# bcgsc/NanoSim

Measured on AMD Instinct MI355X. Metric: simulated reads/sec (genome mode, mean 8 kb), higher is better.
Workload: dtype u8

## Files before the change

### nanosim_amd/csrc/nanosim_amd.hip

```cpp
#include <hip/hip_runtime.h>
#include <hipcub/hipcub.hpp>
#include <stdio.h>
#include <stdlib.h>
#include <string.h>
#include <algorithm>
#include <chrono>
#include <atomic>
#include <condition_variable>
#include <functional>
#include <mutex>
#include <thread>
#include <string>
#include <vector>

#include "ns_device.h"
#include "ns_materialise.h"
#include "ns_chain.h"
#include "ns_hp.h"
#include "ns_ir.h"
#include "ns_io.h"
#include "ns_pack.h"
#include "ns_cs_hist.h"

#ifndef NS_WPB
// ... 1065 lines not shown
        const ns_piece p = A.pieces[gp];
        const uint32_t kind = uni(p.kind);
        const uint32_t out_len = (HPF && !kind) ? uni(A.hp_len[gp]) : uni(p.out_len);
        qualities_piece(A.m, Q, ro, key, a, kind ? NS_GAP_SEG + (pi >> 1) : (pi >> 1), kind, out_len, q, cls + (q >> 4) + 2u * pi, lane);
        q += out_len;
    }
    if (A.polya) {
        const uint32_t pl = uni(A.polya[r]);
        if (pl) emit_polya_quals(A.m, ro, key, a, q, pl, rd.head, rd.tail, lane);
    }
}

#define NS_DENSE_SEG 4096u
__global__ void __launch_bounds__(256) k_dense_plan(GenArgs A, uint32_t *cnt) {
    const uint64_t r = (uint64_t)blockIdx.x * blockDim.x + threadIdx.x;
    if (r > A.prm.n_reads) return;
    uint32_t c = 0;
    if (r < A.prm.n_reads) { const ns_read rd = A.reads[r]; c = rd.flags ? 0u : max(1u, (rd.seq_len + NS_DENSE_SEG - 1u) / NS_DENSE_SEG); }
    cnt[r] = c;
}
template <bool FASTQ>
__global__ void __launch_bounds__(64) k_materialise_dense(GenArgs A, const uint32_t *__restrict__ seg_off) {
    __shared__ DenseLds S;
    const uint32_t lane = threadIdx.x;
    const uint32_t w = blockIdx.x, n = (uint32_t)A.prm.n_reads;
    if (w >= seg_off[n]) return;
    uint32_t lo = 0, hi = n;
    while (hi - lo > 1) { const uint32_t mid = (lo + hi) >> 1; if (seg_off[mid] <= w) lo = mid; else hi = mid; }
    const uint64_t r = uni(lo);
    const uint32_t seg = uni(w - seg_off[lo]);
    ns_read rd; ns_key key; ReadOut ro;
    if (!load_read_uniform(A, r, FASTQ, rd, key, ro)) return;
    const uint32_t a = rd.attempts;
    if (seg == 0) emit_head_tail(A.m, ro, key, a, rd.head, rd.tail, lane);
    uint32_t q = rd.head;
    for (uint32_t pi = 0; pi < rd.n_pieces; ++pi) {
        const PieceCtx pc = load_piece_uniform(A.events, A.ref, A.pieces[rd.piece_off + pi], pi);
        const uint64_t s_lo = (uint64_t)seg * NS_DENSE_SEG, s_hi = s_lo + NS_DENSE_SEG, p_lo = q - rd.head, p_hi = p_lo + pc.out_len;
        if (p_hi > s_lo && p_lo < s_hi) {
            const uint32_t m_lo = (uint32_t)(max(s_lo, p_lo) - p_lo), m_hi = (uint32_t)(min(s_hi, p_hi) - p_lo);
            if (A.dbg & 16384u) slow_piece_range(A.m, A.ref, ro, key, a, pc, q, m_lo, m_hi, lane);
            else dense_piece<FASTQ>(A.m, A.ref, S, ro, key, a, pc, q, m_lo, m_hi, lane);
        }
        q += pc.out_len;
    }
}

template <bool FASTQ, bool SCRATCH>
__global__ void __launch_bounds__(64) k_materialise_slow(GenArgs A, SlowQueue sq) {
    const uint32_t lane = threadIdx.x;
    const uint32_t n = min(*sq.count, sq.cap);
    for (uint32_t i = blockIdx.x; i < n; i += gridDim.x) {
        const SlowTile t = sq.items[i];
        ns_read rd; ns_key key; ReadOut ro;
        if (!load_read_uniform(A, t.read, FASTQ && !SCRATCH, rd, key, ro)) continue;
        uint32_t q = SCRATCH ? 0u : rd.head;
        if constexpr (SCRATCH) { ro.seq = A.scr + A.scr_off[t.read]; ro.qual = nullptr; ro.reversed = false; ro.uracil = false; }
        for (uint32_t pi = 0; pi < t.piece; ++pi) q += A.pieces[rd.piece_off + pi].out_len;
        const PieceCtx pc = load_piece_uniform(A.events, A.ref, A.pieces[rd.piece_off + t.piece], t.piece);
        slow_piece_range<FASTQ && SCRATCH>(A.m, A.ref, ro, key, rd.attempts, pc, q, t.m0, t.m1, lane);
    }
}

template <bool FASTQ>
__global__ void __launch_bounds__(64) k_materialise_slow_hpf(GenArgs A, SlowQueue sq) {
    const uint32_t lane = threadIdx.x;
// ... 407 lines not shown
}

__global__ void __launch_bounds__(64 * NS_WPB) k_errlen(GenArgs A) {
    const uint32_t lane = threadIdx.x & 63;
    const uint64_t r = (uint64_t)blockIdx.x * (blockDim.x >> 6) + (threadIdx.x >> 6);
    if (r >= A.prm.n_reads) return;
    const ns_read rd = A.reads[r];
    unsigned long long sum = 0;
    if (!rd.flags) {
        const uint32_t nl = A.name_len[r];
        for (uint32_t pi = 0; pi < rd.n_pieces; ++pi) {
            const ns_piece p = A.pieces[rd.piece_off + pi];
            if (p.kind) continue;
            const ns_event *ev = A.events + p.ev_off;
            for (uint32_t j = lane; j < p.n_ev; j += 64) {
                const ns_event e = ev[j];
                sum += nl + dec_digits(e.pos) + dec_digits(ns_ev_len(e.info)) + 2u * ns_ev_len(e.info) + 9u;
            }
        }
    }
    sum = wave_sum(sum);
    if (lane == 0) A.err_len[r] = sum;
}

#define NS_ERR_BUF_SMALL 5120u
#define NS_ERR_BUF_LARGE 8192u
#define NS_ERR_PAD 16u
#define NS_ERR_NAME 256u
#define NS_ERR_NAME_ROW (NS_ERR_NAME + 8u)
template <uint32_t BUF>
__global__ void __launch_bounds__(64) k_errlog(GenArgs A) {
    __shared__ __align__(16) uint8_t buf_lds[NS_ERR_PAD + BUF + 16];
    __shared__ __align__(16) uint8_t name_lds[4][NS_ERR_NAME_ROW];
    const uint32_t lane = threadIdx.x & 63;
    const uint64_t r = blockIdx.x;
    if (r >= A.prm.n_reads) return;
    const ns_read rd = A.reads[r];
    if (rd.flags) return;
    const ns_key key = read_key(A, r);
    const uint32_t a = rd.attempts;
    const uint32_t nl = A.name_len[r];
    const uint8_t *name = A.records + rd.rec_off + 1;
    const bool name_in_lds = nl <= NS_ERR_NAME;
    if (name_in_lds) {
        for (uint32_t j = lane; 4u * j < nl + 4u; j += 64) {
            uint32_t v0 = 0;
            for (uint32_t b = 0; b < 4; ++b) if (4u * j + b < nl) v0 |= (uint32_t)name[4u * j + b] << (8 * b);
            const uint32_t vp = j ? (uint32_t)name[4u * j - 1] | (uint32_t)name[4u * j - 2] << 8 | (uint32_t)name[4u * j - 3] << 16 : 0u;
            *reinterpret_cast<uint32_t *>(&name_lds[0][4u * j]) = v0;
            *reinterpret_cast<uint32_t *>(&name_lds[1][4u * j]) = v0 << 8 | (vp & 0xffu);
            *reinterpret_cast<uint32_t *>(&name_lds[2][4u * j]) = v0 << 16 | (vp & 0xffu) << 8 | ((vp >> 8) & 0xffu);
            *reinterpret_cast<uint32_t *>(&name_lds[3][4u * j]) = v0 << 24 | (vp & 0xffu) << 16 | ((vp >> 8) & 0xffu) << 8 | (vp >> 16);
        }
        wave_sync();
    }
    uint64_t base = A.err_off[r];
    for (uint32_t pi = 0; pi < rd.n_pieces; pi += 2) {
        const ns_piece p = A.pieces[rd.piece_off + pi];
        PieceCtx pc = load_piece(A.events, A.ref, p, pi);
        ns_event e_nx; e_nx.pos = 0; e_nx.info = 0;
        if (lane < p.n_ev) e_nx = pc.ev[p.n_ev - 1 - lane];
        for (uint32_t j0 = 0; j0 < p.n_ev; j0 += 64) {
            const uint32_t k = j0 + lane;
            const bool active = k < p.n_ev;
            const ns_event e = e_nx;
            const uint32_t len = ns_ev_len(e.info), ty = ns_ev_type(e.info);
            const uint32_t tail = dec_digits(e.pos) + dec_digits(len) + 2u * len + 9u;
            const uint32_t row = active ? nl + tail : 0;
            const uint32_t incl = wave_incl_scan(row);
            const uint32_t total = (uint32_t)__builtin_amdgcn_readlane((int)incl, 63);
            const bool staged = name_in_lds && total <= BUF;
            auto fields = [&](auto w) __attribute__((always_inline)) {
                if (A.dbg & (1u << 17)) return;
                *w++ = '\t'; w = put_dec_p(w, e.pos); *w++ = '\t';
                const char *tn = ty == NS_MIS ? "mis" : ty == NS_INS ? "ins" : "del";
                *w++ = (uint8_t)tn[0]; *w++ = (uint8_t)tn[1]; *w++ = (uint8_t)tn[2];
                *w++ = '\t'; w = put_dec_p(w, len); *w++ = '\t';
                auto w2 = w + len + 1;
                if (A.dbg & (1u << 18)) return;
                const bool need_ref = ty != NS_INS;
                const bool inside = pc.pos + e.pos + 16ull <= pc.chrom_len;
                uint32_t r16[4] = {0x2d2d2d2du, 0x2d2d2d2du, 0x2d2d2d2du, 0x2d2d2d2du}, n16[4] = {0x2d2d2d2du, 0x2d2d2d2du, 0x2d2d2d2du, 0x2d2d2d2du};
                if (need_ref && inside) __builtin_memcpy(r16, A.ref.bases + pc.chrom_base + pc.pos + e.pos, 16);
                bool fast = len <= 16u && (!need_ref || inside);
                if (fast && need_ref) {
                    const uint32_t nb = 8u * (len & 3u), full = len >> 2;
                    uint32_t amb = 0;
#pragma unroll
                    for (uint32_t g = 0; g < 4; ++g) amb |= r16[g] & (g < full ? 0x80808080u : g == full ? (0x80808080u & ((1u << nb) - 1u)) : 0u);
                    fast = amb == 0;
                }
                if (ty != NS_DEL) {
                    const uint32_t word = payload_word(key, pc.sid, a, p.n_ev - 1 - k, 0);
                    uint32_t f3 = word;
#pragma unroll
                    for (uint32_t g = 0; g < 4; ++g) {
                        if (ty == NS_INS) {
                            const uint32_t x8 = (word >> (8u * g)) & 0xffu, t8 = (x8 | x8 << 12) & 0x000f000fu;
                            n16[g] = __builtin_amdgcn_perm(0u, 0x47435441u, (t8 | t8 << 6) & 0x03030303u);
                        } else {
                            const uint32_t d0 = next_digit3(f3), d1 = next_digit3(f3), d2 = next_digit3(f3), d3 = next_digit3(f3);
                            const uint32_t d4 = d0 | d1 << 8 | d2 << 16 | d3 << 24;
                            const uint32_t vv = (r16[g] >> 1) & 0x03030303u;
                            const uint32_t rank4 = (vv & 0x01010101u) << 1 | ((vv >> 1) & 0x01010101u);
                            const uint32_t ge = ((d4 | 0x80808080u) - rank4) & 0x80808080u;
                            n16[g] = __builtin_amdgcn_perm(0u, 0x47435441u, d4 + (ge >> 7));
                        }
                    }
                }
#pragma unroll
                for (uint32_t i = 0; i < 16; ++i) {
                    const bool on = fast && i < len;
                    if (!__ballot(on)) break;
                    if (on) { w[i] = (uint8_t)(r16[i >> 2] >> (8u * (i & 3u))); w2[i] = (uint8_t)(n16[i >> 2] >> (8u * (i & 3u))); }
                }
                if (!fast) {
                    uint32_t frac = 0;
                    for (uint32_t i = 0; i < len; ++i) {
                        if (ty != NS_DEL && !(i & 15u)) frac = payload_word(key, pc.sid, a, p.n_ev - 1 - k, i >> 4);
                        if (ty == NS_INS) { w[i] = '-'; w2[i] = bases_atcg((frac >> (2u * (i & 15u))) & 3u); }
                        else {
                            uint32_t x = e.pos + i;
                            uint8_t cur = resolve_base((uint32_t)ref_base_at(A.ref, pc, x), key, pc.sid, a, x);
                            w[i] = cur;
                            w2[i] = (ty == NS_MIS) ? mis_from_digit(cur, next_digit3(frac)) : (uint8_t)'-';
                        }
                    }
                }
                w[len] = '\t';
                w2[len] = '\n';
            };
            if (staged) {
                uint8_t *const dst0 = A.errlog + base;
                const uint32_t mis = (uint32_t)(uintptr_t)dst0 & 15u;
                if (active) {
// ... 344 lines not shown
    }
    uint32_t *hist = (uint32_t *)ctx->ord_bins.p, *cursor = hist + NS_ORD_BINS;
    const unsigned tiles = (unsigned)((n + 1023) / 1024);
    if (!tiles) return NS_OK;
    HIPCHK(hipMemsetAsync(hist, 0, NS_ORD_BINS * 4, st));
    k_order_hist<<<dim3(std::min(tiles, 256u)), dim3(1024), 0, st>>>(keys, (uint32_t)n, hist);
    k_order_scan<<<dim3(1), dim3(1024), 0, st>>>(hist, cursor);
    k_order_deal<<<dim3(tiles), dim3(1024), 0, st>>>(keys, (uint32_t)n, cursor, list);
    HIPCHK(hipGetLastError());
    return NS_OK;
}
static void fold_stats(ns_ctx *ctx, hipStream_t st) {
    uint32_t *z = ctx->slow_q.cap >= 16 ? (uint32_t *)ctx->slow_q.p : nullptr;
    k_stats_fold<<<dim3(1), dim3(64), 0, st>>>((unsigned long long *)ctx->stats.p, z);
    ctx->sq_zeroed = z != nullptr;
}
static int read_small(ns_ctx *ctx, hipStream_t st, void *dst, const void *src, size_t n, void *dst2 = nullptr, const void *src2 = nullptr, size_t n2 = 0) {
    if (n > (dst2 ? 512u : 1024u) || n2 > 512) return fail(ctx, NS_EINVAL, "read_small: too large");
    HIPCHK(hipMemcpyAsync(ctx->pin_small, src, n, hipMemcpyDeviceToHost, st));
    if (dst2) HIPCHK(hipMemcpyAsync(ctx->pin_small + 512, src2, n2, hipMemcpyDeviceToHost, st));
    HIPCHK(hipStreamSynchronize(st));
    memcpy(dst, ctx->pin_small, n);
    if (dst2) memcpy(dst2, ctx->pin_small + 512, n2);
    return NS_OK;
}

static void free_pool(std::vector<void *> &pool) {
    for (void *p : pool) { hipError_t e = hipFree(p); (void)e; }
    pool.clear();
}

void ns_destroy(ns_ctx *ctx) {
    if (!ctx) return;
    if (ctx->step) {
        { std::lock_guard<std::mutex> lk(ctx->step->mu); ctx->step->quit = true; }
        ctx->step->cv.notify_all();
        if (ctx->step->th.joinable()) ctx->step->th.join();
        delete ctx->step; ctx->step = nullptr;
    }
    if (ctx->companion) { ns_destroy(ctx->companion); ctx->companion = nullptr; }
    if (ctx->borrowed) {
        ctx->model_allocs.clear(); ctx->ref_allocs.clear(); ctx->ir_allocs.clear(); ctx->ref_bases_owned = nullptr;
        ctx->species_chrom_off = DevBuf{}; ctx->trx_chrom = DevBuf{}; ctx->trx_cum = DevBuf{}; ctx->trx_polya = DevBuf{};
    }
    hipError_t e = hipSetDevice(ctx->device); (void)e;
    if (ctx->io) { ctx->io->wait_all(); ctx->io->shutdown(); delete ctx->io; ctx->io = nullptr; }
    for (ns_sink *s : ctx->sinks) delete s;
    ctx->sinks.clear();
    if (ctx->stream) { e = hipStreamSynchronize(ctx->stream); e = hipStreamDestroy(ctx->stream); }
    if (ctx->stream2) { e = hipStreamSynchronize(ctx->stream2); e = hipStreamDestroy(ctx->stream2); }
    if (ctx->stream3) { e = hipStreamSynchronize(ctx->stream3); e = hipStreamDestroy(ctx->stream3); }
    if (ctx->ev_join3) e = hipEventDestroy(ctx->ev_join3);
    if (ctx->ev_fork) e = hipEventDestroy(ctx->ev_fork);
    if (ctx->ev_join) e = hipEventDestroy(ctx->ev_join);
    free_pool(ctx->model_allocs);
    free_pool(ctx->ref_allocs);
    free_pool(ctx->ir_allocs);
    if (ctx->ref_bases_owned) e = hipFree(ctx->ref_bases_owned);
    DevBuf *bufs[] = {&ctx->n_pieces, &ctx->piece_off, &ctx->ev_cap, &ctx->ev_off, &ctx->rec_len, &ctx->rec_off,
                      &ctx->err_len, &ctx->err_off, &ctx->name_len, &ctx->reads, &ctx->pieces, &ctx->events,
                      &ctx->rec_slot[0], &ctx->rec_slot[1], &ctx->err_slot[0], &ctx->err_slot[1], &ctx->stats, &ctx->scan_tmp, &ctx->sort_key, &ctx->sort_idx, &ctx->ord_bins,
                      &ctx->sort_key_out, &ctx->order, &ctx->list_b, &ctx->list_c, &ctx->rstate, &ctx->att_base, &ctx->scr, &ctx->hp_nev, &ctx->hp_ev, &ctx->hp_wd, &ctx->hp_runs, &ctx->hp_nrun,
                      &ctx->scr_len, &ctx->scr_off, &ctx->hp_len, &ctx->slow_q, &ctx->l_cap, &ctx->l_off, &ctx->species_chrom_off, &ctx->t_reads, &ctx->t_pieces,
                      &ctx->t_name_len, &ctx->t_rec_len, &ctx->t_err_len, &ctx->accept, &ctx->accept_scan, &ctx->key_pos,
                      &ctx->draw_x, &ctx->m_segptr, &ctx->m_len, &ctx->m_species, &ctx->species_bases, &ctx->draw_sel,
                      &ctx->draw_sorted, &ctx->meta_words, &ctx->meta_num, &ctx->trx_chrom, &ctx->trx_cum, &ctx->trx_polya, &ctx->polya,
// ... 1618 lines not shown
```

### nanosim_amd/csrc/ns_device.h

```cpp
#pragma once
#include "ns_rng.h"
#include "../../include/nanosim_amd.h"

struct ChainTab {
    uint32_t n_words;
    uint32_t trans;
    uint32_t mix_w;
    uint32_t mix_rec;
    uint32_t fm_hi, fm_vhi, fm_n, fm_guide;
    uint32_t mm_gv;
    uint32_t pm_lut;
    uint32_t sub2;
    uint32_t pm_bin;
    uint32_t n_words_lds;
    uint32_t fm_gv, mm_gv_full, pm_full, sub2_full;
    uint32_t mm_g16;
    uint32_t int_image;
    uint32_t tail_bits;
    uint32_t n_words_mix;
    uint32_t mm_nbins, mm_bin, mm_bin_lut, mm_seg_off, mm_hi, mm_vhi, mm_vlo0, mm_guide;
    double fm_vlo0;
};

struct DevModel {
// ... 250 lines not shown
NS_DEV uint8_t normalise_base(uint32_t c) {
    c &= 0x7fu;
    if (c >= 'a' && c <= 'z') c -= 32;
    uint32_t n;
    if (is_acgt(c)) return (uint8_t)c;
    iupac_members(c, n);
    return (uint8_t)((n ? c : (uint32_t)'N') | 0x80u);
}
NS_DEV uint8_t resolve_base(uint32_t c, const ns_key &key, uint32_t seg, uint32_t attempt, uint32_t x) {
    if (!(c & 0x80u)) return (uint8_t)c;
    c &= 0x7fu;
    uint32_t n, mem = iupac_members(c, n);
    if (!n) return (uint8_t)c;
    u32x4 w = ns_draw(key, ST_IUPAC, seg, attempt, x >> 2, 0);
    uint32_t j = (uint32_t)(((uint64_t)ns_word(w, x & 3) * n) >> 32);
    return (uint8_t)(mem >> (8 * j));
}
NS_DEV uint32_t payload_word(const ns_key &key, uint32_t seg, uint32_t attempt, uint32_t j, uint32_t c) {
    if (c == 0) { u32x4 w = ns_draw(key, ST_SUB, seg, attempt, j >> 2, 0); return ns_word(w, j & 3); }
    u32x4 w = ns_draw(key, ST_INS, seg, attempt, j, c >> 2);
    return ns_word(w, c & 3);
}
NS_DEV uint8_t mis_from_digit(uint32_t cur, uint32_t dg) {
    int rc = base_rank(cur);
    uint32_t rk = dg + ((int)dg >= rc ? 1u : 0u);
    if (rc < 0) rk = dg;
    return bases_atcg(rk);
}
NS_DEV uint32_t next_digit3(uint32_t &frac) {
    uint64_t p = (uint64_t)frac * 3u;
    frac = (uint32_t)p;
    return (uint32_t)(p >> 32);
}
__device__ __forceinline__ uint8_t mis_letter(uint32_t cur, const ns_key &key, uint32_t seg, uint32_t attempt, uint32_t j, uint32_t i) {
    uint32_t frac = payload_word(key, seg, attempt, j, i >> 4), dg = 0;
    for (uint32_t t = 0; t <= (i & 15); ++t) dg = next_digit3(frac);
    return mis_from_digit(cur, dg);
}
__device__ __forceinline__ uint8_t ins_letter(const ns_key &key, uint32_t seg, uint32_t attempt, uint32_t j, uint32_t i) {
    return bases_atcg((payload_word(key, seg, attempt, j, i >> 4) >> (2 * (i & 15))) & 3u);
}
__device__ __forceinline__ uint8_t ht_letter(const ns_key &key, uint32_t stream, uint32_t attempt, uint32_t i) {
    u32x4 w = ns_draw(key, stream, 0, attempt, i >> 6, 0);
    return bases_atcg((ns_word(w, (i >> 4) & 3) >> (2 * (i & 15))) & 3u);
}
NS_DEV uint8_t qual_value_lut(const uint32_t *__restrict__ thr, const uint16_t *__restrict__ lut, uint32_t h) {
    const uint32_t e = lut[h >> 6];
    if (!(e & 0x8000u)) return (uint8_t)(((e & 0x7fffu) + (h & 63u)) >> 7);
    uint32_t q = (e >> 7) & 0x7fu;
    while (q < NS_QUAL_LEVELS - 1 && h >= thr[q]) ++q;
    return (uint8_t)q;
}
NS_DEV uint8_t qual_value(const uint32_t *__restrict__ thr, uint32_t h) {
    uint32_t lo = 0, hi = NS_QUAL_LEVELS - 1;
    while (lo < hi) {
        uint32_t mid = (lo + hi) >> 1;
        if (h >= thr[mid]) lo = mid + 1; else hi = mid;
    }
    return (uint8_t)lo;
}
__device__ __forceinline__ uint8_t qual_at(const DevModel &m, int cls, const ns_key &key, uint32_t stream, uint32_t seg,
                                           uint32_t attempt, uint32_t mpos) {
    u32x4 w = ns_draw(key, stream, seg, attempt, mpos >> 3, 0);
    uint32_t h = (ns_word(w, (mpos & 7) >> 1) >> (16 * (mpos & 1))) & 0xffffu;
    return qual_value(m.qual_thr + cls * NS_QUAL_LEVELS, h);
}
// ... 30 lines not shown
```

### nanosim_amd/csrc/ns_materialise.h

```cpp
#pragma once
#include "ns_device.h"

#ifndef NS_TILE_CHUNKS
#define NS_TILE_CHUNKS 2u
#endif
#define T_OUT (1024u * NS_TILE_CHUNKS)
#define T_EV 64u
#define T_DUMP (T_OUT + 16u)
#define NS_CLS_MIS_BIT 0x08u
#define NS_CLS_INS_BIT 0x20u
#define NS_CLS_STRIP 0xd7d7d7d7u
#define NS_QLUT_SLOTS 5u
__device__ __forceinline__ uint32_t wave_incl_scan(uint32_t v) {
    v += (uint32_t)__builtin_amdgcn_update_dpp(0, (int)v, 0x111, 0xf, 0xf, true);
    v += (uint32_t)__builtin_amdgcn_update_dpp(0, (int)v, 0x112, 0xf, 0xf, true);
    v += (uint32_t)__builtin_amdgcn_update_dpp(0, (int)v, 0x114, 0xf, 0xf, true);
    v += (uint32_t)__builtin_amdgcn_update_dpp(0, (int)v, 0x118, 0xf, 0xf, true);
    v += (uint32_t)__builtin_amdgcn_update_dpp(0, (int)v, 0x142, 0xa, 0xf, false);
    v += (uint32_t)__builtin_amdgcn_update_dpp(0, (int)v, 0x143, 0xc, 0xf, false);
    return v;
}

__device__ __forceinline__ uint32_t wave_incl_max(uint32_t v) {
    v = max(v, (uint32_t)__builtin_amdgcn_update_dpp(0, (int)v, 0x111, 0xf, 0xf, false));
// ... 282 lines not shown
        }
        store_chunk(ro, pq + m0, count, lo, hi, qlo, qhi);
    }
}

__device__ __forceinline__ void wave_sync() {
    __builtin_amdgcn_fence(__ATOMIC_ACQ_REL, "wavefront");
    __builtin_amdgcn_wave_barrier();
}

typedef __attribute__((address_space(3))) volatile uint8_t *LdsBytes;
typedef __attribute__((address_space(3))) volatile uint32_t *LdsWords;
__device__ __forceinline__ void lds_put_bytes(LdsBytes d, uint32_t x0, uint32_t x1, uint32_t x2, uint32_t x3, uint32_t cn) {
    const uint32_t head = min(cn, (0u - (uint32_t)(uintptr_t)d) & 3u);
    if (head > 0) d[0] = (uint8_t)x0;
    if (head > 1) d[1] = (uint8_t)(x0 >> 8);
    if (head > 2) d[2] = (uint8_t)(x0 >> 16);
    const uint32_t sh = 8u * head;
    const uint32_t y0 = __builtin_amdgcn_alignbit(x1, x0, sh), y1 = __builtin_amdgcn_alignbit(x2, x1, sh), y2 = __builtin_amdgcn_alignbit(x3, x2, sh), y3 = x3 >> sh;
    const uint32_t rem = cn - head;
    const LdsWords w = (LdsWords)(d + head);
    if (rem >= 4u) w[0] = y0;
    if (rem >= 8u) w[1] = y1;
    if (rem >= 12u) w[2] = y2;
    if (rem >= 16u) w[3] = y3;
    const uint32_t yt = rem >= 12u ? y3 : rem >= 8u ? y2 : rem >= 4u ? y1 : y0, tail = rem & 3u;
    const LdsBytes e = d + head + (rem & ~3u);
    if (tail > 0) e[0] = (uint8_t)yt;
    if (tail > 1) e[1] = (uint8_t)(yt >> 8);
    if (tail > 2) e[2] = (uint8_t)(yt >> 16);
}

#define NS_DENSE_TILE 1024u
struct __align__(16) DenseLds { uint8_t out[NS_DENSE_TILE + 64]; };

template <bool FASTQ>
__device__ inline void dense_piece(const DevModel &m, const DevRef &ref, DenseLds &S, const ReadOut &ro, const ns_key &key, uint32_t a,
                                   const PieceCtx &pc, uint32_t pq, uint32_t m_lo, uint32_t m_hi, uint32_t lane) {
    if (m_lo & 15u) { slow_piece_range(m, ref, ro, key, a, pc, pq, m_lo, m_hi, lane); return; }
    const uint32_t n_items = pc.n_ev + 1u;
    const uint8_t *seg0 = ref.bases + pc.chrom_base + pc.pos;
    const uint64_t lin = pc.chrom_len - pc.pos;
    uint32_t jb = 0;
    if (m_lo) {
        uint32_t lo = 0, hi = pc.n_ev;
        while (lo < hi) { const uint32_t mid = (lo + hi) >> 1; if (ev_out_start(pc.ev[mid]) <= m_lo) lo = mid + 1; else hi = mid; }
        jb = uni(lo);
    }
    for (uint32_t M0 = m_lo; M0 < m_hi; M0 += NS_DENSE_TILE) {
        const uint32_t M1 = min(M0 + NS_DENSE_TILE, m_hi);
        uint32_t seen = 0;
        for (uint32_t jj0 = jb;; jj0 += 64) {
            const uint32_t jj = jj0 + lane;
            const bool valid = jj < n_items;
            uint32_t os = 0, pl = 0, ty = 3, rp = 0, pos = 0, nxt = pc.out_len;
            if (valid) {
                if (jj) {
                    const ns_event e = pc.ev[jj - 1];
                    const uint32_t len = ns_ev_len(e.info);
                    ty = ns_ev_type(e.info); os = ev_out_start(e); pos = e.pos;
                    pl = ty == NS_DEL ? 0u : len; rp = e.pos + (ty == NS_INS ? 0u : len);
                }
                if (jj < pc.n_ev) nxt = ev_out_start(pc.ev[jj]);
            }
            const uint32_t lo = max(os, M0), hi = min(nxt, M1);
            const bool act = valid && lo < hi;
            const uint32_t n_let = act ? min(pl, hi - os) : 0u;
            const uint32_t c_lo = max(lo, os + pl);
            const uint32_t cn = act && c_lo < hi ? hi - c_lo : 0u;
            const uint32_t x0 = rp + (c_lo - os - pl);
            const bool fast_l = n_let && os >= M0 && (ty == NS_INS || (uint64_t)pos + n_let <= lin);
            bool fast_c = cn && cn <= 16u && (uint64_t)x0 + 16u <= lin;
            uint4 f = make_uint4(0, 0, 0, 0);
            if (fast_c) __builtin_memcpy(&f, seg0 + x0, 16);
            if ((f.x | f.y | f.z | f.w) & 0x80808080u) fast_c = false;
            {
                uint32_t nl_max = fast_l ? n_let : 0u;
                nl_max = max(nl_max, (uint32_t)__builtin_amdgcn_update_dpp(0, (int)nl_max, 0x111, 0xf, 0xf, false));
                nl_max = max(nl_max, (uint32_t)__builtin_amdgcn_update_dpp(0, (int)nl_max, 0x112, 0xf, 0xf, false));
                nl_max = max(nl_max, (uint32_t)__builtin_amdgcn_update_dpp(0, (int)nl_max, 0x114, 0xf, 0xf, false));
                nl_max = max(nl_max, (uint32_t)__builtin_amdgcn_update_dpp(0, (int)nl_max, 0x118, 0xf, 0xf, false));
                const uint32_t m01 = max((uint32_t)__builtin_amdgcn_readlane((int)nl_max, 15), (uint32_t)__builtin_amdgcn_readlane((int)nl_max, 31));
                const uint32_t m23 = max((uint32_t)__builtin_amdgcn_readlane((int)nl_max, 47), (uint32_t)__builtin_amdgcn_readlane((int)nl_max, 63));
                const uint32_t groups = (max(m01, m23) + 3u) >> 2;
                uint32_t frac = 0;
                const uint32_t o_base = os - M0;
                for (uint32_t g = 0; g < groups; ++g) {
                    const uint32_t i0 = 4u * g;
                    const bool on = fast_l && i0 < n_let;
                    if (!(g & 3u) && on) frac = payload_word(key, pc.sid, a, jj - 1u, g >> 2);
                    uint32_t cur4 = 0x41414141u;
                    if (on && ty != NS_INS) {
                        __builtin_memcpy(&cur4, seg0 + pos + i0, 4);
                        if (cur4 & 0x80808080u) {
                            uint32_t rs = 0;
                            for (uint32_t t = 0; t < 4u; ++t) rs |= (uint32_t)resolve_base((cur4 >> (8u * t)) & 0xffu, key, pc.sid, a, pos + i0 + t) << (8u * t);
                            cur4 = rs;
                        }
                    }
                    const uint32_t x8 = (frac >> (8u * (g & 3u))) & 0xffu, t8 = (x8 | x8 << 12) & 0x000f000fu;
                    const uint32_t ins4 = __builtin_amdgcn_perm(0u, 0x47435441u, (t8 | t8 << 6) & 0x03030303u);
                    uint32_t f3 = frac;
                    const uint32_t d0 = next_digit3(f3), d1 = next_digit3(f3), d2 = next_digit3(f3), d3 = next_digit3(f3);
                    const uint32_t d4 = d0 | d1 << 8 | d2 << 16 | d3 << 24;
                    const uint32_t vv = (cur4 >> 1) & 0x03030303u;
                    const uint32_t rank4 = (vv & 0x01010101u) << 1 | ((vv >> 1) & 0x01010101u);
                    const uint32_t ge = ((d4 | 0x80808080u) - rank4) & 0x80808080u;
                    const uint32_t mis4 = __builtin_amdgcn_perm(0u, 0x47435441u, d4 + (ge >> 7));
                    const bool is_ins = ty == NS_INS;
                    if (!is_ins) frac = f3;
                    const uint32_t letters = is_ins ? ins4 : mis4;
                    const uint32_t cnt = on ? n_let - i0 : 0u, dump = NS_DENSE_TILE + lane, o = o_base + i0;
                    S.out[cnt > 0 ? o : dump] = (uint8_t)letters; S.out[cnt > 1 ? o + 1 : dump] = (uint8_t)(letters >> 8);
                    S.out[cnt > 2 ? o + 2 : dump] = (uint8_t)(letters >> 16); S.out[cnt > 3 ? o + 3 : dump] = (uint8_t)(letters >> 24);
                }
            }
            if (fast_c) lds_put_bytes((LdsBytes)&S.out[c_lo - M0], f.x, f.y, f.z, f.w, cn);
            if (act && ((n_let && !fast_l) || (cn && !fast_c))) {
                if (!fast_l) {
                    uint32_t word = 0;
                    for (uint32_t i = 0; i < n_let; ++i) {
                        if (!(i & 15u)) word = payload_word(key, pc.sid, a, jj - 1u, i >> 4);
                        uint32_t b;
                        if (ty == NS_INS) b = bases_atcg((word >> (2u * (i & 15u))) & 3u);
                        else {
                            const uint32_t x = pos + i;
                            b = mis_from_digit(resolve_base(ref_base_at(ref, pc, x), key, pc.sid, a, x), next_digit3(word));
                        }
                        if (os + i >= lo) S.out[os + i - M0] = (uint8_t)b;
                    }
                }
                if (cn && !fast_c) {
                    for (uint32_t i = 0; i < cn; ++i) {
                        const uint32_t x = x0 + i;
                        S.out[c_lo + i - M0] = resolve_base(ref_base_at(ref, pc, x), key, pc.sid, a, x);
                    }
                }
            }
            seen += (uint32_t)__popcll(__ballot(valid && os <= M1));
            if (__ballot(valid && os >= M1) || jj0 + 64u >= n_items) break;
        }
        jb = jb + seen - 1u;
        wave_sync();
        const uint32_t m0 = M0 + 16u * lane;
        if (m0 < M1) {
            const uint32_t count = min(16u, M1 - m0);
            const uint4 v = *reinterpret_cast<const uint4 *>(&S.out[16u * lane]);
// ... 82 lines not shown
    const uint32_t e = (w >> (8u * k)) & 0xffu;
    uint32_t t = e << 3;
    t |= e << 9; t |= e << 15; t |= e << 21;
    return t & 0x18181818u;
}
__device__ __forceinline__ uint64_t cls_word0(uint64_t rec_off, uint64_t r, uint32_t per_read) { return (rec_off >> 4) + r * per_read; }
__device__ __forceinline__ uint32_t cls_per_read(const ns_params &prm) { return prm.chimeric ? 2u * (2u * NS_MAX_SEG - 1u) : 2u; }

__device__ __forceinline__ void qual_lut_load(uint16_t *lds, const DevModel &m, uint32_t tid, uint32_t nthreads) {
    const uint4 *src = reinterpret_cast<const uint4 *>(m.qual_lut);
    uint4 *dst = reinterpret_cast<uint4 *>(lds);
    for (uint32_t i = tid; i < NS_QLUT_SLOTS * 128u; i += nthreads) dst[i] = src[i];
}

__device__ __forceinline__ void lds_or32(uint8_t *p, uint32_t v) {
    __hip_atomic_fetch_or(reinterpret_cast<unsigned int *>(p), v, __ATOMIC_RELAXED, __HIP_MEMORY_SCOPE_WAVEFRONT);
}
__device__ __forceinline__ void lds_or64(uint8_t *p, uint64_t v) {
    __hip_atomic_fetch_or(reinterpret_cast<unsigned long long *>(p), (unsigned long long)v, __ATOMIC_RELAXED, __HIP_MEMORY_SCOPE_WAVEFRONT);
}

template <int MODE>
__device__ __forceinline__ uint32_t event_word(const PieceCtx &pc, const ns_key &key, uint32_t a, uint32_t j) {
    if constexpr (MODE == MAT_HP_FINAL) return pc.wd[j];
    else { const u32x4 w = ns_draw(key, ST_SUB, pc.sid, a, j >> 2, 0); return ns_word(w, j & 3u); }
}
template <uint32_t TC>
struct __align__(16) TileLds7 {
    static constexpr uint32_t T_OUT_ = 1024u * TC;
    uint32_t mlut[17][4];
    uint2 ent[T_EV + 1];
    uint32_t eos[T_EV + 1];
    uint32_t hist[64 * TC];
    __align__(16) uint8_t out[1024u * TC + 16 + 64];
};
template <uint32_t TC>
__device__ __forceinline__ void tile_lds_init(TileLds7<TC> &T, uint32_t lane) {
    for (uint32_t c = lane * 16; c < 1024u * TC + 16 + 64; c += 64 * 16) *reinterpret_cast<uint4 *>(&T.out[c]) = make_uint4(0, 0, 0, 0);
    if (lane < 17) {
#pragma unroll
        for (uint32_t k = 0; k < 4; ++k)
            T.mlut[lane][k] = lane <= 4 * k ? 0xffffffffu : lane >= 4 * k + 4 ? 0u : 0xffffffffu << (8 * (lane - 4 * k));
    }
}
__device__ __forceinline__ void resolve16(uint32_t &a0, uint32_t &a1, uint32_t &a2, uint32_t &a3, uint32_t i0, uint32_t i1, uint32_t x0,
                                          const ns_key &key, uint32_t sid, uint32_t a) {
    for (uint32_t b = i0; b < i1; ++b) {
        uint32_t wk = b < 8 ? (b < 4 ? a0 : a1) : (b < 12 ? a2 : a3);
        const uint32_t ch = (wk >> (8 * (b & 3))) & 0xff;
        if (!(ch & 0x80u)) continue;
        const uint32_t r = resolve_base(ch, key, sid, a, x0 + b);
        wk = (wk & ~(0xffu << (8 * (b & 3)))) | r << (8 * (b & 3));
        if (b < 4) a0 = wk; else if (b < 8) a1 = wk; else if (b < 12) a2 = wk; else a3 = wk;
    }
}
#ifdef NS_ABLATE
#define NS_DBG(bit) (dbg & (bit))
#else
#define NS_DBG(bit) false
#endif
__device__ __forceinline__ uint32_t and_andn(uint32_t a, uint32_t b, uint32_t c) { return __builtin_amdgcn_bitop3_b32(a, b, c, 0x40); }
template <bool FASTQ, int MODE, uint32_t TC>
__device__ inline void materialise_piece7(const DevModel &m, const DevRef &ref, TileLds7<TC> &T, const ReadOut &ro, const ns_key &key,
                                          uint32_t a, const PieceCtx &pc, uint32_t pq, uint32_t lane, uint32_t dbg, const SlowQueue &sq,
                                          uint32_t read_idx, uint32_t piece_idx, uint32_t *__restrict__ cls) {
    constexpr bool CLSOUT = FASTQ && MODE != MAT_HP_SCRATCH;
    constexpr bool HPF = MODE == MAT_HP_FINAL;
    constexpr uint32_t T_OUT_ = 1024u * TC;
    uint32_t jb = 0;
    uint32_t L0_out = 0, L0_rp = 0, L0_pt = 3u << 12, L0_wd = 0, L0_j = 0;
    const uint8_t *seg0 = ref.bases + pc.chrom_base + pc.pos;
    const bool wraps = !HPF && pc.pos + pc.ref_len > pc.chrom_len;
    const uint32_t wrap_at = wraps ? (uint32_t)(pc.chrom_len - pc.pos) : 0xffffffffu;
    const uint32_t phi = ro.reversed ? ((uint32_t)(uintptr_t)ro.seq + ro.seq_len - pq) & 15u : (0u - ((uint32_t)(uintptr_t)ro.seq + pq)) & 15u;
    ns_event e_pre; e_pre.pos = 0; e_pre.info = 0; uint32_t w_pre = 0;
    if (lane < pc.n_ev) e_pre = pc.ev[lane];
    auto cached_word = [&](uint32_t j0) -> uint32_t { if (NS_DBG(64u)) return 0u; const uint32_t j = j0 + lane; return event_word<MODE>(pc, key, a, j < pc.n_ev ? j : 0u); };
    w_pre = cached_word(0u);
    uint32_t cls_carry = 0;
    for (uint32_t M0 = 0; M0 < pc.out_len;) {
        const uint32_t A0 = M0 - ((M0 - phi) & 15u);
        uint32_t M1 = min(A0 + T_OUT_, pc.out_len);
        const ns_event e = e_pre;
        const uint32_t e_wd = w_pre;
        const bool valid = jb + lane < pc.n_ev;
        const uint32_t os = ev_out_start(e), len = ns_ev_len(e.info), ty = ns_ev_type(e.info);
        const uint32_t e_pt = (ty == NS_DEL ? 0u : len) | ty << 12, e_rp = e.pos + (ty == NS_INS ? 0u : len);
        if (jb + 63 < pc.n_ev) {
            const uint32_t os63 = (uint32_t)__builtin_amdgcn_readlane((int)os, 63);
            if (os63 < M1) {
                const uint32_t cut = A0 + ((os63 - A0) & ~15u);
                M1 = (int32_t)(cut - M0) > 0 ? cut : os63;
            }
        }
// ... 75 lines not shown
        uint4 f[TC]; uint32_t fi[TC], fy[TC];
        {
            uint32_t scan_base = 0;
#pragma unroll
            for (uint32_t t = 0; t < TC; ++t) {
                const uint32_t ci = 64 * t + lane;
                const uint32_t incl = max(scan_base, wave_incl_max(T.hist[ci]));
                scan_base = (uint32_t)__builtin_amdgcn_readlane((int)incl, 63);
                f[t] = make_uint4(0, 0, 0, 0); fi[t] = 16u | 16u << 8; fy[t] = 0;
                if (ci < nc && !NS_DBG(1u) && !NS_DBG(256u)) {
                    const uint32_t cs = A0 + 16u * ci, p = ci == 0 ? M0 : cs;
                    const uint2 E = T.ent[incl];
                    const uint32_t nx = T.eos[incl];
                    const uint32_t st = max(p, E.x), en = min(nx, min(cs + 16u, M1));
                    if ((int32_t)(en - st) > 0) {
                        fi[t] = (st - cs) | (en - cs) << 8; fy[t] = E.y;
                        __builtin_memcpy(&f[t], tb + (E.y + cs + 32u), 16);
                    }
                }
            }
        }
        uint4 fe = make_uint4(0, 0, 0, 0); uint32_t ei0 = 16, ei1 = 16, eoc = 0;
        if (take && !NS_DBG(1u) && !NS_DBG(128u)) {
            const uint32_t c = (s1 - A0) >> 4, ecs = A0 + 16u * c;
            const uint32_t en = min(os_next, min(ecs + 16u, M1));
            if ((int32_t)(en - s1) > 0 && ekey > c) {
                eoc = 16u * c; ei0 = s1 - ecs; ei1 = en - ecs;
                __builtin_memcpy(&fe, tb + (y1 + ecs + 32u), 16);
            }
        }
        if (!NS_DBG(2u)) {
            const bool cont = lane == 63 && L0_out + (L0_pt & 0xfffu) > M0;
            const uint32_t b_os = cont ? L0_out : os, b_pt = cont ? L0_pt : e_pt, b_rp = cont ? L0_rp : e_rp;
            const uint32_t b_j = cont ? L0_j : jb + lane;
            uint32_t frac = cont ? L0_wd : e_wd;
            const uint32_t b_pl = b_pt & 0xfffu, b_ty = b_pt >> 12;
            const bool on = (take || cont) && b_pl;
            const uint32_t xs = b_rp - b_pl;
            const bool mis = b_ty == NS_MIS;
            bool fast_l = on && b_pl <= 8 && b_os >= M0 && b_os + b_pl <= M1 && !wraps;
            uint2 cur8 = make_uint2(0x41414141u, 0x41414141u);
            if (fast_l && mis) __builtin_memcpy(&cur8, seg0 + xs, 8);
            if constexpr (!HPF) fast_l = fast_l && !((cur8.x | cur8.y) & 0x80808080u);
            if (fast_l) {
                uint32_t f3 = frac, L2[2];
#pragma unroll
                for (uint32_t g = 0; g < 2; ++g) {
                    const uint32_t cur4 = g ? cur8.y : cur8.x;
                    const uint32_t x8 = (frac >> (8u * g)) & 0xffu, t8 = (x8 | x8 << 12) & 0x000f000fu;
                    const uint32_t ins4 = __builtin_amdgcn_perm(0u, 0x47435441u, (t8 | t8 << 6) & 0x03030303u);
                    const uint32_t d0 = next_digit3(f3), d1 = next_digit3(f3), d2 = next_digit3(f3), d3 = next_digit3(f3);
                    const uint32_t d4 = d0 | d1 << 8 | d2 << 16 | d3 << 24;
                    const uint32_t vv = (cur4 >> 1) & 0x03030303u;
                    const uint32_t rank4 = (vv & 0x01010101u) << 1 | ((vv >> 1) & 0x01010101u);
                    const uint32_t ge = ((d4 | 0x80808080u) - rank4) & 0x80808080u;
                    const uint32_t mis4 = __builtin_amdgcn_perm(0u, 0x47435441u, d4 + (ge >> 7));
                    uint32_t letters = mis ? mis4 : ins4;
                    if constexpr (FASTQ) {
                        uint32_t cls4 = mis ? 0x01010101u * NS_CLS_MIS_BIT : 0x01010101u * NS_CLS_INS_BIT;
                        if constexpr (HPF) {
                            if (mis) cls4 = (frac & 1u) ? NS_CLS_MIS_BIT : (cur4 & (NS_CLS_MIS_BIT | NS_CLS_INS_BIT));
                            else if (g == 0 && (frac >> 31)) cls4 = (cls4 & ~0xffu) | NS_CLS_MIS_BIT;
                        }
                        letters |= cls4;
                    }
                    L2[g] = letters;
                }
                const uint64_t keep = b_pl >= 8u ? ~0ull : ~(~0ull << (8u * b_pl));
                const uint64_t v = ((uint64_t)L2[0] | (uint64_t)L2[1] << 32) & keep;
                const uint32_t o = b_os - A0, sh = 8u * (o & 3u);
                const uint64_t lo64 = v << sh;
                const uint32_t top = (uint32_t)(((v >> 32) << sh) >> 32);
                uint8_t *w = &T.out[o & ~3u];
                lds_or32(w, (uint32_t)lo64); lds_or32(w + 4, (uint32_t)(lo64 >> 32)); lds_or32(w + 8, top);
            }
            if (on && !fast_l) {
                const uint32_t i_lo = b_os < M0 ? M0 - b_os : 0u;
                const uint32_t i_hi = min(b_pl, M1 - b_os);
                const uint32_t word0 = frac;
                for (uint32_t i = 0; i < i_hi; ++i) {
                    if (i && !(i & 15)) frac = payload_word(key, pc.sid, a, b_j, i >> 4);
                    uint32_t b;
                    if (b_ty == NS_INS) {
                        b = bases_atcg((frac >> (2 * (i & 15))) & 3u);
                        if constexpr (FASTQ) b |= (HPF && i == 0 && (word0 >> 31)) ? NS_CLS_MIS_BIT : NS_CLS_INS_BIT;
                    } else {
                        const uint32_t x = xs + i;
                        const uint32_t src = ref_base_at(ref, pc, x);
                        if constexpr (HPF) {
                            b = mis_from_digit(src & ~(NS_CLS_MIS_BIT | NS_CLS_INS_BIT), next_digit3(frac));
                            if constexpr (FASTQ) b |= (word0 & 1u) ? NS_CLS_MIS_BIT : (src & (NS_CLS_MIS_BIT | NS_CLS_INS_BIT));
                        } else {
                            b = mis_from_digit(resolve_base(src, key, pc.sid, a, x), next_digit3(frac));
                            if constexpr (FASTQ) b |= NS_CLS_MIS_BIT;
                        }
                    }
                    if (i >= i_lo) T.out[b_os + i - A0] = (uint8_t)b;
                }
            }
        }
        if (cnt && ei0 < 16u && !NS_DBG(32u)) {
            const uint4 m0 = *reinterpret_cast<const uint4 *>(&T.mlut[ei0][0]), m1 = *reinterpret_cast<const uint4 *>(&T.mlut[ei1][0]);
            uint32_t a0 = and_andn(fe.x, m0.x, m1.x), a1 = and_andn(fe.y, m0.y, m1.y), a2 = and_andn(fe.z, m0.z, m1.z), a3 = and_andn(fe.w, m0.w, m1.w);
            if constexpr (!HPF) {
                if ((a0 | a1 | a2 | a3) & 0x80808080u) resolve16(a0, a1, a2, a3, ei0, ei1, A0 + eoc + y1, key, pc.sid, a);
            }
            lds_or64(&T.out[eoc], (uint64_t)a0 | (uint64_t)a1 << 32);
            lds_or64(&T.out[eoc + 8], (uint64_t)a2 | (uint64_t)a3 << 32);
        }
        wave_sync();
#pragma unroll
        for (uint32_t t = 0; t < TC; ++t) {
            const uint32_t ci = 64 * t + lane;
            const uint32_t c0 = A0 + 16 * ci;
            const uint32_t lo_m = ci == 0 ? M0 : c0, hi_m = min(c0 + 16, M1);
            const bool active = (int32_t)(hi_m - lo_m) > 0 && !NS_DBG(1u);
            uint32_t cw = 0;
            if (active) {
                const uint4 v = *reinterpret_cast<const uint4 *>(&T.out[16 * ci]);
                *reinterpret_cast<uint4 *>(&T.out[16 * ci]) = make_uint4(0, 0, 0, 0);
                const uint32_t i0 = fi[t] & 0xffu, i1 = fi[t] >> 8;
                const uint4 m0 = *reinterpret_cast<const uint4 *>(&T.mlut[i0][0]), m1 = *reinterpret_cast<const uint4 *>(&T.mlut[i1][0]);
                uint32_t a0 = and_andn(f[t].x, m0.x, m1.x), a1 = and_andn(f[t].y, m0.y, m1.y), a2 = and_andn(f[t].z, m0.z, m1.z), a3 = and_andn(f[t].w, m0.w, m1.w);
                if constexpr (!HPF) {
                    if ((a0 | a1 | a2 | a3) & 0x80808080u) resolve16(a0, a1, a2, a3, i0, i1, c0 + fy[t], key, pc.sid, a);
                }
                if (NS_DBG(512u)) { a0 = a1 = a2 = a3 = 0x41414141u; }
                uint32_t r0 = v.x | a0, r1 = v.y | a1, r2 = v.z | a2, r3 = v.w | a3;
                uint64_t qlo = 0, qhi = 0;
                uint32_t s0 = lo_m - c0, count = hi_m - lo_m;
// ... 66 lines not shown
```

Measured before the change: 122.4 million.

## Use LDS base-3 digit table and word-wise letter emission for long events

```diff
diff --git a/nanosim_amd/csrc/nanosim_amd.hip b/nanosim_amd/csrc/nanosim_amd.hip
--- a/nanosim_amd/csrc/nanosim_amd.hip
+++ b/nanosim_amd/csrc/nanosim_amd.hip
@@ -1121,6 +1121,8 @@
     ns_read rd; ns_key key; ReadOut ro;
     if (!load_read_uniform(A, r, FASTQ, rd, key, ro)) return;
     const uint32_t a = rd.attempts;
+    digit3_tab_init(S.dig3, lane);
+    wave_sync();
     if (seg == 0) emit_head_tail(A.m, ro, key, a, rd.head, rd.tail, lane);
     uint32_t q = rd.head;
     for (uint32_t pi = 0; pi < rd.n_pieces; ++pi) {
@@ -1594,6 +1596,7 @@
 __global__ void __launch_bounds__(64) k_errlog(GenArgs A) {
     __shared__ __align__(16) uint8_t buf_lds[NS_ERR_PAD + BUF + 16];
     __shared__ __align__(16) uint8_t name_lds[4][NS_ERR_NAME_ROW];
+    __shared__ uint32_t dig3[NS_DIGIT3_TAB];
     const uint32_t lane = threadIdx.x & 63;
     const uint64_t r = blockIdx.x;
     if (r >= A.prm.n_reads) return;
@@ -1604,6 +1607,8 @@
     const uint32_t nl = A.name_len[r];
     const uint8_t *name = A.records + rd.rec_off + 1;
     const bool name_in_lds = nl <= NS_ERR_NAME;
+    digit3_tab_init(dig3, lane);
+    wave_sync();
     if (name_in_lds) {
         for (uint32_t j = lane; 4u * j < nl + 4u; j += 64) {
             uint32_t v0 = 0;
@@ -1661,8 +1666,7 @@
                             const uint32_t x8 = (word >> (8u * g)) & 0xffu, t8 = (x8 | x8 << 12) & 0x000f000fu;
                             n16[g] = __builtin_amdgcn_perm(0u, 0x47435441u, (t8 | t8 << 6) & 0x03030303u);
                         } else {
-                            const uint32_t d0 = next_digit3(f3), d1 = next_digit3(f3), d2 = next_digit3(f3), d3 = next_digit3(f3);
-                            const uint32_t d4 = d0 | d1 << 8 | d2 << 16 | d3 << 24;
+                            const uint32_t d4 = next_digits3x4(f3, dig3);
                             const uint32_t vv = (r16[g] >> 1) & 0x03030303u;
                             const uint32_t rank4 = (vv & 0x01010101u) << 1 | ((vv >> 1) & 0x01010101u);
                             const uint32_t ge = ((d4 | 0x80808080u) - rank4) & 0x80808080u;
@@ -2073,6 +2077,13 @@
 
 void ns_destroy(ns_ctx *ctx) {
     if (!ctx) return;
+#ifdef NS_ABLATE
+    if (!ctx->borrowed) {
+        unsigned long long c[3] = {0, 0, 0};
+        if (hipMemcpyFromSymbol(c, HIP_SYMBOL(ns_ablate_letter_tiles), sizeof c) == hipSuccess)
+            fprintf(stderr, "NS_ABLATE letter tiles: %llu, into the word loop: %llu, per byte: %llu\n", c[0], c[1], c[2]);
+    }
+#endif
     if (ctx->step) {
         { std::lock_guard<std::mutex> lk(ctx->step->mu); ctx->step->quit = true; }
         ctx->step->cv.notify_all();
diff --git a/nanosim_amd/csrc/ns_device.h b/nanosim_amd/csrc/ns_device.h
--- a/nanosim_amd/csrc/ns_device.h
+++ b/nanosim_amd/csrc/ns_device.h
@@ -306,6 +306,22 @@
     frac = (uint32_t)p;
     return (uint32_t)(p >> 32);
 }
+#define NS_DIGIT3_TAB 81u
+NS_DEV uint32_t digit3_pack4(uint32_t q) {
+    const uint32_t a0 = (q * 19u) >> 9, a1 = (q * 57u) >> 9, a2 = (q * 43u) >> 7;
+    const uint32_t A = a0 | a1 << 8 | a2 << 16 | q << 24;
+    return A - 3u * (A << 8);
+}
+template <class Tab>
+NS_DEV void digit3_tab_init(Tab tab, uint32_t lane) {
+    for (uint32_t q = lane; q < NS_DIGIT3_TAB; q += 64u) tab[q] = digit3_pack4(q);
+}
+template <class Tab>
+NS_DEV uint32_t next_digits3x4(uint32_t &frac, Tab tab) {
+    const uint64_t p = (uint64_t)frac * 81u;
+    frac = (uint32_t)p;
+    return tab[(uint32_t)(p >> 32)];
+}
 __device__ __forceinline__ uint8_t mis_letter(uint32_t cur, const ns_key &key, uint32_t seg, uint32_t attempt, uint32_t j, uint32_t i) {
     uint32_t frac = payload_word(key, seg, attempt, j, i >> 4), dg = 0;
     for (uint32_t t = 0; t <= (i & 15); ++t) dg = next_digit3(frac);
diff --git a/nanosim_amd/csrc/ns_materialise.h b/nanosim_amd/csrc/ns_materialise.h
--- a/nanosim_amd/csrc/ns_materialise.h
+++ b/nanosim_amd/csrc/ns_materialise.h
@@ -338,7 +338,10 @@
 }
 
 #define NS_DENSE_TILE 1024u
-struct __align__(16) DenseLds { uint8_t out[NS_DENSE_TILE + 64]; };
+struct __align__(16) DenseLds {
+    uint8_t out[NS_DENSE_TILE + 64];
+    uint32_t dig3[NS_DIGIT3_TAB + 3];
+};
 
 template <bool FASTQ>
 __device__ inline void dense_piece(const DevModel &m, const DevRef &ref, DenseLds &S, const ReadOut &ro, const ns_key &key, uint32_t a,
@@ -371,11 +374,11 @@
             }
             const uint32_t lo = max(os, M0), hi = min(nxt, M1);
             const bool act = valid && lo < hi;
-            const uint32_t n_let = act ? min(pl, hi - os) : 0u;
+            const uint32_t n_let = act && os + pl > lo ? min(pl, hi - os) : 0u;
             const uint32_t c_lo = max(lo, os + pl);
             const uint32_t cn = act && c_lo < hi ? hi - c_lo : 0u;
             const uint32_t x0 = rp + (c_lo - os - pl);
-            const bool fast_l = n_let && os >= M0 && (ty == NS_INS || (uint64_t)pos + n_let <= lin);
+            const bool fast_l = n_let && (ty == NS_INS || (uint64_t)pos + n_let <= lin);
             bool fast_c = cn && cn <= 16u && (uint64_t)x0 + 16u <= lin;
             uint4 f = make_uint4(0, 0, 0, 0);
             if (fast_c) __builtin_memcpy(&f, seg0 + x0, 16);
@@ -407,8 +410,7 @@
                     const uint32_t x8 = (frac >> (8u * (g & 3u))) & 0xffu, t8 = (x8 | x8 << 12) & 0x000f000fu;
                     const uint32_t ins4 = __builtin_amdgcn_perm(0u, 0x47435441u, (t8 | t8 << 6) & 0x03030303u);
                     uint32_t f3 = frac;
-                    const uint32_t d0 = next_digit3(f3), d1 = next_digit3(f3), d2 = next_digit3(f3), d3 = next_digit3(f3);
-                    const uint32_t d4 = d0 | d1 << 8 | d2 << 16 | d3 << 24;
+                    const uint32_t d4 = next_digits3x4(f3, S.dig3);
                     const uint32_t vv = (cur4 >> 1) & 0x03030303u;
                     const uint32_t rank4 = (vv & 0x01010101u) << 1 | ((vv >> 1) & 0x01010101u);
                     const uint32_t ge = ((d4 | 0x80808080u) - rank4) & 0x80808080u;
@@ -417,8 +419,8 @@
                     if (!is_ins) frac = f3;
                     const uint32_t letters = is_ins ? ins4 : mis4;
                     const uint32_t cnt = on ? n_let - i0 : 0u, dump = NS_DENSE_TILE + lane, o = o_base + i0;
-                    S.out[cnt > 0 ? o : dump] = (uint8_t)letters; S.out[cnt > 1 ? o + 1 : dump] = (uint8_t)(letters >> 8);
-                    S.out[cnt > 2 ? o + 2 : dump] = (uint8_t)(letters >> 16); S.out[cnt > 3 ? o + 3 : dump] = (uint8_t)(letters >> 24);
+                    S.out[cnt > 0 ? min(o, dump) : dump] = (uint8_t)letters; S.out[cnt > 1 ? min(o + 1, dump) : dump] = (uint8_t)(letters >> 8);
+                    S.out[cnt > 2 ? min(o + 2, dump) : dump] = (uint8_t)(letters >> 16); S.out[cnt > 3 ? min(o + 3, dump) : dump] = (uint8_t)(letters >> 24);
                 }
             }
             if (fast_c) lds_put_bytes((LdsBytes)&S.out[c_lo - M0], f.x, f.y, f.z, f.w, cn);
@@ -567,11 +569,13 @@
     uint2 ent[T_EV + 1];
     uint32_t eos[T_EV + 1];
     uint32_t hist[64 * TC];
+    uint32_t dig3[NS_DIGIT3_TAB + 3];
     __align__(16) uint8_t out[1024u * TC + 16 + 64];
 };
 template <uint32_t TC>
 __device__ __forceinline__ void tile_lds_init(TileLds7<TC> &T, uint32_t lane) {
     for (uint32_t c = lane * 16; c < 1024u * TC + 16 + 64; c += 64 * 16) *reinterpret_cast<uint4 *>(&T.out[c]) = make_uint4(0, 0, 0, 0);
+    digit3_tab_init(T.dig3, lane);
     if (lane < 17) {
 #pragma unroll
         for (uint32_t k = 0; k < 4; ++k)
@@ -591,10 +595,43 @@
 }
 #ifdef NS_ABLATE
 #define NS_DBG(bit) (dbg & (bit))
+__device__ unsigned long long ns_ablate_letter_tiles[3];
+#define NS_COUNT_TILE(k) do { if (lane == 0) atomicAdd(&ns_ablate_letter_tiles[k], 1ull); } while (0)
 #else
 #define NS_DBG(bit) false
+#define NS_COUNT_TILE(k) do { } while (0)
 #endif
 __device__ __forceinline__ uint32_t and_andn(uint32_t a, uint32_t b, uint32_t c) { return __builtin_amdgcn_bitop3_b32(a, b, c, 0x40); }
+template <bool FASTQ, bool HPF, uint32_t T_OUT_>
+__device__ __forceinline__ void letter_group(uint8_t *out, const uint32_t *dig3, uint32_t &frac, uint32_t cur4, bool mis, uint32_t word0,
+                                         uint32_t g, uint32_t i0, uint32_t i_hi, uint32_t o0, uint32_t m0r) {
+    const uint32_t x8 = (frac >> (8u * g)) & 0xffu, t8 = (x8 | x8 << 12) & 0x000f000fu;
+    const uint32_t ins4 = __builtin_amdgcn_perm(0u, 0x47435441u, (t8 | t8 << 6) & 0x03030303u);
+    uint32_t f3 = frac;
+    const uint32_t d4 = next_digits3x4(f3, dig3);
+    if (mis) frac = f3;
+    const uint32_t vv = (cur4 >> 1) & 0x03030303u;
+    const uint32_t rank4 = (vv & 0x01010101u) << 1 | ((vv >> 1) & 0x01010101u);
+    const uint32_t ge = ((d4 | 0x80808080u) - rank4) & 0x80808080u;
+    const uint32_t mis4 = __builtin_amdgcn_perm(0u, 0x47435441u, d4 + (ge >> 7));
+    uint32_t letters = mis ? mis4 : ins4;
+    if constexpr (FASTQ) {
+        uint32_t cls4 = mis ? 0x01010101u * NS_CLS_MIS_BIT : 0x01010101u * NS_CLS_INS_BIT;
+        if constexpr (HPF) {
+            if (mis) cls4 = (word0 & 1u) ? 0x01010101u * NS_CLS_MIS_BIT : (cur4 & (0x01010101u * (NS_CLS_MIS_BIT | NS_CLS_INS_BIT)));
+            else if (i0 == 0 && (word0 >> 31)) cls4 = (cls4 & ~0xffu) | NS_CLS_MIS_BIT;
+        }
+        letters |= cls4;
+    }
+    const uint32_t o = o0 + i0, sh = 8u * (o & 3u);
+    uint32_t keep = 0xffffffffu >> (32u - 8u * min(4u, i_hi - i0));
+    const int32_t front = (int32_t)(m0r - o);
+    if (front > 0) keep = front >= 4 ? 0u : keep & (0xffffffffu << (8 * front));
+    const uint32_t v = letters & keep;
+    const uint32_t lo32 = v << sh, hi32 = (v >> 8) >> (24u - sh);
+    const uint32_t ow = o & ~3u, dump = T_OUT_ + 16u;
+    lds_or32(&out[lo32 ? ow : dump], lo32); lds_or32(&out[hi32 ? ow + 4u : dump], hi32);
+}
 template <bool FASTQ, int MODE, uint32_t TC>
 __device__ inline void materialise_piece7(const DevModel &m, const DevRef &ref, TileLds7<TC> &T, const ReadOut &ro, const ns_key &key,
                                           uint32_t a, const PieceCtx &pc, uint32_t pq, uint32_t lane, uint32_t dbg, const SlowQueue &sq,
@@ -736,70 +773,76 @@
         if (!NS_DBG(2u)) {
             const bool cont = lane == 63 && L0_out + (L0_pt & 0xfffu) > M0;
             const uint32_t b_os = cont ? L0_out : os, b_pt = cont ? L0_pt : e_pt, b_rp = cont ? L0_rp : e_rp;
-            const uint32_t b_j = cont ? L0_j : jb + lane;
             uint32_t frac = cont ? L0_wd : e_wd;
             const uint32_t b_pl = b_pt & 0xfffu, b_ty = b_pt >> 12;
             const bool on = (take || cont) && b_pl;
             const uint32_t xs = b_rp - b_pl;
             const bool mis = b_ty == NS_MIS;
-            bool fast_l = on && b_pl <= 8 && b_os >= M0 && b_os + b_pl <= M1 && !wraps;
+            const uint32_t i_hi = on ? min(b_pl, M1 - b_os) : 0u;
+            const uint32_t m0r = M0 - A0;
+            const uint32_t word0 = HPF ? frac : 0u;
+            const uint32_t o0 = b_os - A0;
+            constexpr uint32_t NO_PB = 0xffffffffu;
+            uint32_t pb = wraps ? 0u : NO_PB;
             uint2 cur8 = make_uint2(0x41414141u, 0x41414141u);
-            if (fast_l && mis) __builtin_memcpy(&cur8, seg0 + xs, 8);
-            if constexpr (!HPF) fast_l = fast_l && !((cur8.x | cur8.y) & 0x80808080u);
-            if (fast_l) {
-                uint32_t f3 = frac, L2[2];
-#pragma unroll
-                for (uint32_t g = 0; g < 2; ++g) {
-                    const uint32_t cur4 = g ? cur8.y : cur8.x;
-                    const uint32_t x8 = (frac >> (8u * g)) & 0xffu, t8 = (x8 | x8 << 12) & 0x000f000fu;
-                    const uint32_t ins4 = __builtin_amdgcn_perm(0u, 0x47435441u, (t8 | t8 << 6) & 0x03030303u);
-                    const uint32_t d0 = next_digit3(f3), d1 = next_digit3(f3), d2 = next_digit3(f3), d3 = next_digit3(f3);
-                    const uint32_t d4 = d0 | d1 << 8 | d2 << 16 | d3 << 24;
-                    const uint32_t vv = (cur4 >> 1) & 0x03030303u;
-                    const uint32_t rank4 = (vv & 0x01010101u) << 1 | ((vv >> 1) & 0x01010101u);
-                    const uint32_t ge = ((d4 | 0x80808080u) - rank4) & 0x80808080u;
-                    const uint32_t mis4 = __builtin_amdgcn_perm(0u, 0x47435441u, d4 + (ge >> 7));
-                    uint32_t letters = mis ? mis4 : ins4;
-                    if constexpr (FASTQ) {
-                        uint32_t cls4 = mis ? 0x01010101u * NS_CLS_MIS_BIT : 0x01010101u * NS_CLS_INS_BIT;
-                        if constexpr (HPF) {
-                            if (mis) cls4 = (frac & 1u) ? NS_CLS_MIS_BIT : (cur4 & (NS_CLS_MIS_BIT | NS_CLS_INS_BIT));
-                            else if (g == 0 && (frac >> 31)) cls4 = (cls4 & ~0xffu) | NS_CLS_MIS_BIT;
-                        }
-                        letters |= cls4;
-                    }
-                    L2[g] = letters;
-                }
-                const uint64_t keep = b_pl >= 8u ? ~0ull : ~(~0ull << (8u * b_pl));
-                const uint64_t v = ((uint64_t)L2[0] | (uint64_t)L2[1] << 32) & keep;
-                const uint32_t o = b_os - A0, sh = 8u * (o & 3u);
-                const uint64_t lo64 = v << sh;
-                const uint32_t top = (uint32_t)(((v >> 32) << sh) >> 32);
-                uint8_t *w = &T.out[o & ~3u];
-                lds_or32(w, (uint32_t)lo64); lds_or32(w + 4, (uint32_t)(lo64 >> 32)); lds_or32(w + 8, top);
-            }
-            if (on && !fast_l) {
-                const uint32_t i_lo = b_os < M0 ? M0 - b_os : 0u;
-                const uint32_t i_hi = min(b_pl, M1 - b_os);
-                const uint32_t word0 = frac;
-                for (uint32_t i = 0; i < i_hi; ++i) {
-                    if (i && !(i & 15)) frac = payload_word(key, pc.sid, a, b_j, i >> 4);
-                    uint32_t b;
-                    if (b_ty == NS_INS) {
-                        b = bases_atcg((frac >> (2 * (i & 15))) & 3u);
-                        if constexpr (FASTQ) b |= (HPF && i == 0 && (word0 >> 31)) ? NS_CLS_MIS_BIT : NS_CLS_INS_BIT;
-                    } else {
-                        const uint32_t x = xs + i;
-                        const uint32_t src = ref_base_at(ref, pc, x);
-                        if constexpr (HPF) {
-                            b = mis_from_digit(src & ~(NS_CLS_MIS_BIT | NS_CLS_INS_BIT), next_digit3(frac));
-                            if constexpr (FASTQ) b |= (word0 & 1u) ? NS_CLS_MIS_BIT : (src & (NS_CLS_MIS_BIT | NS_CLS_INS_BIT));
-                        } else {
-                            b = mis_from_digit(resolve_base(src, key, pc.sid, a, x), next_digit3(frac));
-                            if constexpr (FASTQ) b |= NS_CLS_MIS_BIT;
+            if (pb == NO_PB && i_hi) {
+                if (mis) {
+                    __builtin_memcpy(&cur8, seg0 + xs, 8);
+                    if constexpr (!HPF) { if ((cur8.x | cur8.y) & 0x80808080u) pb = 0u; }
+                }
+                if (pb == NO_PB) letter_group<FASTQ, HPF, T_OUT_>(T.out, T.dig3, frac, cur8.x, mis, word0, 0u, 0u, i_hi, o0, m0r);
+            }
+            if (__ballot(pb == NO_PB && i_hi > 4u)) {
+                if (pb == NO_PB && i_hi > 4u) letter_group<FASTQ, HPF, T_OUT_>(T.out, T.dig3, frac, cur8.y, mis, word0, 1u, 4u, i_hi, o0, m0r);
+            }
+            NS_COUNT_TILE(0);
+            if (__builtin_expect(__ballot(i_hi > 8u || (pb != NO_PB && i_hi)) != 0, 0)) {
+                NS_COUNT_TILE(1);
+#ifdef NS_ABLATE
+                bool counted = false;
+#endif
+                for (uint32_t c = 0;; ++c) {
+                    const bool won = 16u * c < i_hi;
+                    if (!__ballot(won)) break;
+                    if (c && won) { const u32x4 w = ns_draw(key, ST_INS, pc.sid, a, cont ? L0_j : jb + lane, c >> 2); frac = ns_word(w, c & 3u); }
+#pragma unroll 1
+                    for (uint32_t g = c ? 0u : 2u; g < 4u; ++g) {
+                        const uint32_t i0 = 16u * c + 4u * g;
+                        if (!__ballot(pb == NO_PB && i0 < i_hi)) break;
+                        if (pb == NO_PB && i0 < i_hi) {
+                            uint32_t cur4 = 0x41414141u;
+                            if (mis) {
+                                __builtin_memcpy(&cur4, seg0 + xs + i0, 4);
+                                if constexpr (!HPF) { if (cur4 & 0x80808080u) pb = i0; }
+                            }
+                            if (pb == NO_PB) letter_group<FASTQ, HPF, T_OUT_>(T.out, T.dig3, frac, cur4, mis, word0, g, i0, i_hi, o0, m0r);
                         }
                     }
-                    if (i >= i_lo) T.out[b_os + i - A0] = (uint8_t)b;
+#ifdef NS_ABLATE
+                    if (!counted && __ballot(won && pb != NO_PB)) { NS_COUNT_TILE(2); counted = true; }
+#endif
+                    if (won && pb != NO_PB) {
+                        const uint32_t i_end = min(16u * c + 16u, i_hi);
+                        for (uint32_t i = pb; i < i_end; ++i) {
+                            uint32_t b;
+                            if (!mis) {
+                                b = bases_atcg((frac >> (2 * (i & 15))) & 3u);
+                                if constexpr (FASTQ) b |= (HPF && i == 0 && (word0 >> 31)) ? NS_CLS_MIS_BIT : NS_CLS_INS_BIT;
+                            } else {
+                                const uint32_t x = xs + i;
+                                const uint32_t src = ref_base_at(ref, pc, x);
+                                if constexpr (HPF) {
+                                    b = mis_from_digit(src & ~(NS_CLS_MIS_BIT | NS_CLS_INS_BIT), next_digit3(frac));
+                                    if constexpr (FASTQ) b |= (word0 & 1u) ? NS_CLS_MIS_BIT : (src & (NS_CLS_MIS_BIT | NS_CLS_INS_BIT));
+                                } else {
+                                    b = mis_from_digit(resolve_base(src, key, pc.sid, a, x), next_digit3(frac));
+                                    if constexpr (FASTQ) b |= NS_CLS_MIS_BIT;
+                                }
+                            }
+                            if ((int32_t)(o0 + i - m0r) >= 0) T.out[o0 + i] = (uint8_t)b;
+                        }
+                        pb = i_end;
+                    }
                 }
             }
         }
```

After: 121.4 million. No clear change (-0.8%).
